# udaysankar01/xfeatSLAM

Hardware: AMD Instinct MI355X
Metric: XFeat frames/s (VGA, 4096 kpts) + 4096x4096 desc-match pairs/s (higher is better)
Workload: dtype f32

## Files before the change

xfeatslam_amd/csrc/capi.cpp:

```cpp
#include "host_stage.h"

#include <dlfcn.h>
#include <math.h>
#include <stdio.h>
#include <stdlib.h>
#include <string.h>
#include <vector>

int conv_layer_npart(int li, int Hout, int Wout);

namespace {
struct Roctx {
    int (*push)(const char*) = nullptr;
    int (*pop)() = nullptr;
};
Roctx* roctx() {
    static Roctx* R = []() -> Roctx* {
        const char* e = getenv("XFH_ROCTX");
        if (!e || !*e || *e == '0') return nullptr;
        static Roctx r;
        for (const char* n : {"librocprofiler-sdk-roctx.so.1", "librocprofiler-sdk-roctx.so", "libroctx64.so.4", "libroctx64.so"}) {
            void* h = dlopen(n, RTLD_NOW | RTLD_GLOBAL);
            if (!h) continue;
            *(void**)(&r.push) = dlsym(h, "roctxRangePushA");
// ... 136 lines not shown
            }
        }
#endif
        if (masked) {
            if (hipExtStreamCreateWithCUMask(&c->own_stream, 8, mask) != hipSuccess) return fail(XFH_ERR_HIP);
            if (hipExtStreamCreateWithCUMask(&c->aux_stream, 8, mask) != hipSuccess) return fail(XFH_ERR_HIP);
        } else {
            if (hipStreamCreateWithFlags(&c->own_stream, hipStreamNonBlocking) != hipSuccess) return fail(XFH_ERR_HIP);
            if (hipStreamCreateWithFlags(&c->aux_stream, hipStreamNonBlocking) != hipSuccess) return fail(XFH_ERR_HIP);
        }
    }
    c->stream = c->own_stream;
    if (hipEventCreateWithFlags(&c->ev_fork, hipEventDisableTiming) != hipSuccess) return fail(XFH_ERR_HIP);
    if (hipEventCreateWithFlags(&c->ev_join, hipEventDisableTiming) != hipSuccess) return fail(XFH_ERR_HIP);
    if (hipEventCreateWithFlags(&c->ev_out, hipEventDisableTiming) != hipSuccess) return fail(XFH_ERR_HIP);
    const size_t xs = (size_t)c->Hmax * c->Wmax;
    A(c->d_gray, (size_t)B * cfg->max_height * cfg->max_width);
    A(c->X, sizeof(float) * B * xs);
    c->pre_npart = (int)((xs + 1023) / 1024);
    A(c->pre_part, sizeof(double) * B * c->pre_npart * 2);
    A(c->xstat, sizeof(float) * B * 2);
    int lh[XFH_NUM_LAYERS], lw[XFH_NUM_LAYERS];
    layer_dims(c->Hmax, c->Wmax, lh, lw);
    for (int i = 0; i < XFH_NUM_LAYERS; ++i) {
        const int C = XFH_LAYERS[i].cout;
        c->raw_stride[i] = (size_t)lh[i] * lw[i] * C;
        if (i != 0) A(c->raw[i], sizeof(float) * B * c->raw_stride[i]);
        c->part_stride[i] = (size_t)conv_layer_npart(i, lh[i], lw[i]) * C * 2;
        A(c->part[i], sizeof(double) * B * c->part_stride[i]);
        A(c->stat[i], sizeof(float) * B * 2 * C);
    }
    A(c->skip_pool, sizeof(float) * B * (xs / 16));
    A(c->feats, sizeof(float) * B * c->raw_stride[17]);
    if (B > 32) { A(c->act4, sizeof(float) * B * c->raw_stride[11]); A(c->act5, sizeof(float) * B * c->raw_stride[15]); }
    A(c->feat_nrm, sizeof(float) * B * (xs / 64));
    A(c->H1, sizeof(float) * B * (xs / 64));
    A(c->K1h, sizeof(float) * B * xs);
    c->cand_cap = 1024;
    while (c->cand_cap < xs) c->cand_cap <<= 1;
    A(c->cand, sizeof(u64) * B * c->cand_cap);
    A(c->cand_count, sizeof(int) * B * CAND_CNT_STRIDE);
    A(c->slot_src, sizeof(int) * B * cfg->nfeatures);
    A(c->sel_key, sizeof(u64) * B * cfg->nfeatures);
    A(c->sel_n, sizeof(int) * B);
    const size_t rec = xfh_record_bytes(cfg->nfeatures);
    A(c->d_records, rec * B);
    if (hipHostMalloc((void**)&c->h_records, rec, hipHostMallocDefault) != hipSuccess) return fail(XFH_ERR_OUT_OF_MEMORY);
    if (hipHostMalloc((void**)&c->h_gray, (size_t)cfg->max_height * cfg->max_width, hipHostMallocDefault) != hipSuccess) return fail(XFH_ERR_OUT_OF_MEMORY);
    c->s_hgray[0] = c->h_gray; c->s_dgray[0] = c->d_gray; c->s_hrec[0] = c->h_records;
    for (int k = 1; k < xfh_ctx::SLOTS; ++k) {
        A(c->s_dgray[k], (size_t)cfg->max_height * cfg->max_width);
        if (hipHostMalloc((void**)&c->s_hgray[k], (size_t)cfg->max_height * cfg->max_width, hipHostMallocDefault) != hipSuccess) return fail(XFH_ERR_OUT_OF_MEMORY);
        if (hipHostMalloc((void**)&c->s_hrec[k], rec, hipHostMallocDefault) != hipSuccess) return fail(XFH_ERR_OUT_OF_MEMORY);
    }
    for (int k = 0; k < xfh_ctx::SLOTS; ++k)
        if (hipEventCreateWithFlags(&c->s_done[k], hipEventDisableTiming) != hipSuccess) return fail(XFH_ERR_HIP);
#undef A
    if (match_ws_reserve(c, cfg->nfeatures, cfg->nfeatures) != hipSuccess) return fail(XFH_ERR_OUT_OF_MEMORY);
    if (HostStage::reserve(c, match_mnn_stage_bytes(cfg->nfeatures, cfg->nfeatures)) != XFH_OK) return fail(XFH_ERR_OUT_OF_MEMORY);
    c->mws.cap_hout = (size_t)cfg->nfeatures * 12 + 256;
    if (hipHostMalloc((void**)&c->mws.h_out, c->mws.cap_hout, hipHostMallocDefault) != hipSuccess) return fail(XFH_ERR_OUT_OF_MEMORY);
    if (hipStreamSynchronize(c->stream) != hipSuccess) return fail(XFH_ERR_HIP);
    if (xfh_verbose()) fprintf(stderr, "[xfh] ctx %p: device %d, %dx%d (x32: %dx%d), nfeatures %d, max_batch %d, bn_mode %d, flags %d\n", (void*)c, cfg->device,
                               cfg->max_height, cfg->max_width, c->Hmax, c->Wmax, cfg->nfeatures, cfg->max_batch, cfg->bn_mode, cfg->flags);
    *out = c;
    return XFH_OK;
}

int xfh_destroy(xfh_ctx* c) {
    if (!c) return XFH_OK;
    hipSetDevice(c->cfg.device);
    if (c->twin) { xfh_destroy(c->twin); c->twin = nullptr; }
    pipe_destroy(c);
    xfh_comm_destroy(c);
    if (c->stream && c->stream != c->own_stream) hipStreamSynchronize(c->stream);
    if (c->own_stream) hipStreamSynchronize(c->own_stream);
    if (c->aux_stream) hipStreamSynchronize(c->aux_stream);
    auto F = [](void* p) { if (p) hipFree(p); };
    F(c->d_gray); F(c->X); F(c->pre_part); F(c->xstat);
    for (int i = 0; i < XFH_NUM_LAYERS; ++i) { F(c->raw[i]); F(c->part[i]); F(c->stat[i]); }
    if (!c->is_twin && !c->is_lane) {
        for (int i = 0; i < XFH_NUM_LAYERS; ++i) { F(c->w.mfma[i]); F(c->w.alt[i]); F(c->w.alt2[i]); F(c->w.m16[i]); F(c->w.bn_bias[i]); }
        for (int i = 0; i < 3; ++i) F(c->w.direct[i]);
        F(c->w.fus2); F(c->w.fus2_bias); F(c->w.skip_w); F(c->w.skip_b); F(c->w.heat2_w); F(c->w.heat2_b); F(c->w.kp3_w); F(c->w.kp3_b);
    }
    F(c->skip_pool); F(c->feats); F(c->act4); F(c->act5); F(c->feat_nrm); F(c->H1); F(c->K1h);
    F(c->cand); F(c->cand_count); F(c->slot_src); F(c->sel_key); F(c->sel_n); F(c->d_records);
    if (c->h_records) hipHostFree(c->h_records);
    if (c->h_gray) hipHostFree(c->h_gray);
    for (int k = 1; k < xfh_ctx::SLOTS; ++k) { F(c->s_dgray[k]); if (c->s_hgray[k]) hipHostFree(c->s_hgray[k]); if (c->s_hrec[k]) hipHostFree(c->s_hrec[k]); }
    for (int k = 0; k < xfh_ctx::SLOTS; ++k) if (c->s_done[k]) hipEventDestroy(c->s_done[k]);
    MatchWs& w = c->mws;
    F(w.img1); F(w.keys); F(w.stage); F(w.bkeys);
    if (w.h_out) hipHostFree(w.h_out);
    if (c->timer.ev) { for (int i = 0; i < 2 * KTimer::MAXEV; ++i) if (c->timer.ev[i]) hipEventDestroy(c->timer.ev[i]); free(c->timer.ev); }
    if (c->ev_fork) hipEventDestroy(c->ev_fork);
    if (c->ev_join) hipEventDestroy(c->ev_join);
    if (c->ev_out) hipEventDestroy(c->ev_out);
    if (c->aux_stream) hipStreamDestroy(c->aux_stream);
    if (c->own_stream) hipStreamDestroy(c->own_stream);
    delete c;
    return XFH_OK;
}

struct BlobEntry { const float* p; uint32_t dims[4]; uint32_t ndim; };
static bool blob_find(const void* blob, size_t nbytes, const char* name, BlobEntry* e) {
    const unsigned char* p = (const unsigned char*)blob;
    if (nbytes < 16 || memcmp(p, "XFHWGT01", 8) != 0) return false;
    uint32_t n; memcpy(&n, p + 8, 4);
    const size_t esz = 48 + 4 + 16 + 8;
    if (16 + (size_t)n * esz > nbytes) return false;
    const unsigned char* data = p + 16 + (size_t)n * esz;
    for (uint32_t i = 0; i < n; ++i) {
        const unsigned char* q = p + 16 + (size_t)i * esz;
        if (strncmp((const char*)q, name, 48) == 0) {
            memcpy(&e->ndim, q + 48, 4); memcpy(e->dims, q + 52, 16);
            uint64_t off; memcpy(&off, q + 68, 8);
            if (e->ndim > 4) return false;
            const uint64_t total = (nbytes - (size_t)(data - p)) / 4;
// ... 290 lines not shown
```

xfeatslam_amd/csrc/ctx.h:

```cpp
#pragma once
#include "common.h"
#include <hip/hip_ext.h>
#include <atomic>
#include <string>

struct DevWeights {
    float* direct[3] = {nullptr, nullptr, nullptr};
    float* mfma[XFH_NUM_LAYERS] = {};
    float* alt2[XFH_NUM_LAYERS] = {};
    float* m16[XFH_NUM_LAYERS] = {};
    float* alt[XFH_NUM_LAYERS] = {};
    float* bn_bias[XFH_NUM_LAYERS] = {};
    float* fus2 = nullptr;
    float* fus2_bias = nullptr;
    float* skip_w = nullptr; float* skip_b = nullptr;
    float* heat2_w = nullptr; float* heat2_b = nullptr;
    float* kp3_w = nullptr; float* kp3_b = nullptr;
    bool loaded = false;
};

struct XfhComm;
struct xfh_ctx;

#define XFH_PIPE_MAX_LANES 8
// ... 13 lines not shown
    bool inline_busy = false;
    int b_head = 0, b_count = 0;
};

struct xfh_ctx {
    xfh_config cfg;
    XfhComm* comm = nullptr;
    int Hmax = 0, Wmax = 0;
    int num_cu = 256;
    hipStream_t own_stream = nullptr;
    hipStream_t stream = nullptr;
    hipStream_t aux_stream = nullptr;
    hipEvent_t ev_fork = nullptr, ev_join = nullptr;
    hipEvent_t ev_out = nullptr;
    std::string hip_err;

    DevWeights w;

    int B = 0, H0 = 0, W0 = 0, H = 0, W = 0;
    int lh[XFH_NUM_LAYERS] = {}, lw[XFH_NUM_LAYERS] = {};
    int npart[XFH_NUM_LAYERS] = {};
    unsigned long long written[2] = {0ull, 0ull};

    uint8_t* d_gray = nullptr;
    float* X = nullptr;
    double* pre_part = nullptr; int pre_npart = 0;
    float* xstat = nullptr;
    float* raw[XFH_NUM_LAYERS] = {};
    double* part[XFH_NUM_LAYERS] = {};
    float* stat[XFH_NUM_LAYERS] = {};
    size_t raw_stride[XFH_NUM_LAYERS] = {};
    size_t part_stride[XFH_NUM_LAYERS] = {};
    float* skip_pool = nullptr; float* feats = nullptr;
    float* act4 = nullptr; float* act5 = nullptr;
    float* H1 = nullptr; float* K1h = nullptr;
    bool no_nms_heat = false;
    bool no_ride = false;
    bool select_legacy = false;
    float* feat_nrm = nullptr;
    u64* cand = nullptr; size_t cand_cap = 0;
    int* cand_count = nullptr;
    int* slot_src = nullptr;
    u64* sel_key = nullptr;
    int* sel_n = nullptr;
    uint8_t* d_records = nullptr;
    uint8_t* h_records = nullptr;
    uint8_t* h_gray = nullptr;

    static const int SLOTS = 2;
    uint8_t* s_hgray[SLOTS] = {}; uint8_t* s_dgray[SLOTS] = {}; uint8_t* s_hrec[SLOTS] = {};
    hipEvent_t s_done[SLOTS] = {};
    xfh_ctx* twin = nullptr;
    bool is_twin = false;
    int s_head = 0, s_count = 0;

    Pipe pipe;
    bool is_lane = false;

    MatchWs mws;
    KTimer timer;
};

void xfh_trace_push(const char* name);
void xfh_trace_pop();
bool xfh_verbose();
struct XfhRange { explicit XfhRange(const char* n) { xfh_trace_push(n); } ~XfhRange() { xfh_trace_pop(); } };

// ... 32 lines not shown
```

xfeatslam_amd/csrc/kernels_conv.hip:

```cpp
#include "ctx.h"
#include "heads_kp4.hip.h"
#include <stdlib.h>

struct ConvArgs {
    const float* in;
    StatSrc st;
    size_t in_stride;
    int Hin, Win;
    const float* w;
    const float* bias;
    float* out;
    size_t out_stride;
    int Hout, Wout;
    double* part;
    size_t part_stride;
    int tiles_x;
    const float* pool; size_t pool_stride; const float* skip_w; const float* skip_b;
    const float* r4; size_t s4; int H4, W4; StatSrc st4;
    const float* r5; size_t s5; int H5, W5; StatSrc st5;
    const float* xstat; const float* w0; const float* bias0;
    int dbg;
};

enum { PRO_PLAIN = 0, PRO_BN = 1, PRO_IN = 2, PRO_B2IN = 3, PRO_FUSE = 4, PRO_L0 = 5, PRO_UNFOLD = 6, PRO_FUSEA = 7  };
enum { EPI_STATS = 0, EPI_BIAS = 1, EPI_BIAS_RELU = 2 };

#ifdef XFH_STAMPS
__device__ unsigned long long g_stamps[32 * 8];
#define XFH_STAMP(a, ph) do { if (blockIdx.x == gridDim.x / 2 && blockIdx.y == 0 && blockIdx.z == 0 && threadIdx.x == 0) g_stamps[((a).dbg & 31) * 8 + (ph)] = wall_clock64(); } while (0)
extern "C" int xfh_debug_stamps(unsigned long long* out) { return (int)hipMemcpyFromSymbol(out, HIP_SYMBOL(g_stamps), sizeof g_stamps); }
#define XFH_STAMP_ROW(row, ph) do { if (blockIdx.x == gridDim.x / 2 && blockIdx.y == 0 && blockIdx.z == 0 && threadIdx.x == 0) g_stamps[(row) * 8 + (ph)] = wall_clock64(); } while (0)
#else
#define XFH_STAMP(a, ph) do { } while (0)
#define XFH_STAMP_ROW(row, ph) do { } while (0)
#endif

__device__ __forceinline__ void lin_coeff_c(int in, int out, int d, int& i0, int& i1, float& l0, float& l1) {
    const float scale = (float)in / (float)out;
    float src = fmaf(scale, (float)d + 0.5f, -0.5f);
    if (src < 0.f) src = 0.f;
    int a = (int)src;
    if (a > in - 1) a = in - 1;
    float lam = src - (float)a;
    lam = fminf(fmaxf(lam, 0.f), 1.f);
    i0 = a; i1 = a + ((a < in - 1) ? 1 : 0);
    l1 = lam; l0 = 1.f - lam;
}
template <bool ACT = false>
__device__ __forceinline__ void ld_act8(const float* __restrict__ raw, const float* st, size_t pix, int g, f32x4& v0, f32x4& v1) {
    const float* p = raw + pix * 64 + g * 8;
    v0 = *(const f32x4*)p; v1 = *(const f32x4*)(p + 4);
    if constexpr (ACT) return;
#pragma unroll
    for (int q = 0; q < 4; ++q) {
        v0[q] = fmaxf(fmaf(v0[q], st[64 + g * 8 + q], st[g * 8 + q]), 0.f);
        v1[q] = fmaxf(fmaf(v1[q], st[64 + g * 8 + 4 + q], st[g * 8 + 4 + q]), 0.f);
    }
}
template <bool ACT = false>
__device__ __forceinline__ void up_bilinear8(const float* __restrict__ raw, const float* st, int Hi, int Wi, int Ho, int Wo, int y, int x, int g, f32x4& o0, f32x4& o1) {
    int y0, y1, x0, x1; float hy0, hy1, wx0, wx1;
    lin_coeff_c(Hi, Ho, y, y0, y1, hy0, hy1);
    lin_coeff_c(Wi, Wo, x, x0, x1, wx0, wx1);
    f32x4 a0, a1, b0, b1, c0, c1, d0, d1;
    ld_act8<ACT>(raw, st, (size_t)y0 * Wi + x0, g, a0, a1); ld_act8<ACT>(raw, st, (size_t)y0 * Wi + x1, g, b0, b1);
    ld_act8<ACT>(raw, st, (size_t)y1 * Wi + x0, g, c0, c1); ld_act8<ACT>(raw, st, (size_t)y1 * Wi + x1, g, d0, d1);
#pragma unroll
    for (int j = 0; j < 4; ++j) {
        const float t0 = fmaf(wx0, a0[j], wx1 * b0[j]), u0 = fmaf(wx0, c0[j], wx1 * d0[j]);
        o0[j] = fmaf(hy0, t0, hy1 * u0);
        const float t1 = fmaf(wx0, a1[j], wx1 * b1[j]), u1 = fmaf(wx0, c1[j], wx1 * d1[j]);
        o1[j] = fmaf(hy0, t1, hy1 * u1);
    }
}

__global__ __launch_bounds__(256)
void k_act_pyramid(const float* __restrict__ raw4, size_t s4, const float* __restrict__ st4, int n4 ,
                   const float* __restrict__ raw5, size_t s5, const float* __restrict__ st5, int n5, float* __restrict__ act4, float* __restrict__ act5) {
    const int b = blockIdx.z;
    for (int q = blockIdx.x * 256 + threadIdx.x; q < (n4 + n5) / 4; q += gridDim.x * 256) {
        const bool five = q >= n4 / 4;
        const int e = (five ? q - n4 / 4 : q) * 4, ch = e & 63;
        const float* st = (five ? st5 : st4) + (size_t)b * 128;
        const size_t off = (size_t)b * (five ? s5 : s4) + e;
        f32x4 v = *(const f32x4*)((five ? raw5 : raw4) + off);
        const f32x4 be = *(const f32x4*)(st + ch), al = *(const f32x4*)(st + 64 + ch);
#pragma unroll
        for (int j = 0; j < 4; ++j) v[j] = fmaxf(fmaf(v[j], al[j], be[j]), 0.f);
        *(f32x4*)((five ? act5 : act4) + off) = v;
    }
}

__global__ __launch_bounds__(256)
void k_bn_finalize(const double* __restrict__ part, size_t part_stride, int npart, int C, double count,
                   float* __restrict__ stat ) {
    __shared__ double red[256 * 2];
    const int b = blockIdx.x;
    bn_fold<16>(part + (size_t)b * part_stride, npart, C, count, stat + (size_t)b * 2 * C, red, threadIdx.x, 256);
}

__device__ __forceinline__ double wave_sum_f64(double v) {
    v += __shfl_xor(v, 32); v += __shfl_xor(v, 16); v += __shfl_xor(v, 8);
    v += __shfl_xor(v, 4); v += __shfl_xor(v, 2); v += __shfl_xor(v, 1);
    return v;
}
typedef float f32x2 __attribute__((ext_vector_type(2)));
__device__ __forceinline__ void l0_conv(const float (&win)[9], const XFH_CONST float* __restrict__ w, float (&acc)[4]) {
    f32x2 a0 = {0.f, 0.f}, a1 = {0.f, 0.f};
#pragma unroll
    for (int k = 0; k < 9; ++k) {
        const f32x2 v = {win[k], win[k]};
        a0 = __builtin_elementwise_fma(v, f32x2{w[k * 4], w[k * 4 + 1]}, a0);
        a1 = __builtin_elementwise_fma(v, f32x2{w[k * 4 + 2], w[k * 4 + 3]}, a1);
    }
    acc[0] = a0.x; acc[1] = a0.y; acc[2] = a1.x; acc[3] = a1.y;
}

constexpr int L0S_TW = 128, L0S_TH = 32, L0S_R = 4;
__global__ __launch_bounds__(256)
void k_block1_stats(const float* __restrict__ X, size_t x_stride, StatSrc xs, int H, int W, int tiles_x,
                    const float* __restrict__ w0, double* __restrict__ part, size_t part_stride, float* __restrict__ pool, size_t pool_stride) {
    __shared__ double s_red[512];
    __shared__ float s_xst[2];
// ... 304 lines not shown
            if (cok && prow < rows_left && pcol + 4 * h < cols_left) value(n, r, dst, bv);
        }
    }
}

#ifndef XFH_PD
#define XFH_PD 3
#endif

template <int CIN, int COUT, int KS, int ST, int WM, int WN, int NT, int WW, int PRO, int EPI, int CBMAX = 64, int TPC = 1, int PD = XFH_PD>
__device__ __forceinline__ void conv_mfma_body(const ConvArgs a, const int tile, const int b, float* smem) {
    constexpr int NTHR = 64 * WM * WN;
    constexpr int WH = 32 / WW, TH = WM * WH, TW = WW;
    constexpr int COUTP = WN * NT * 32;
    constexpr int PAD = KS / 2;
    constexpr int TIH = (TH - 1) * ST + KS, TIW = (TW - 1) * ST + KS;
    constexpr int CP = CIN + 4;
    constexpr int CB = CIN > CBMAX ? CBMAX : CIN;
    constexpr int NCB = CIN / CB;
    static_assert(TPC == 1 || NCB == 1, "several taps per chunk only with all channels in the chunk");
    static_assert((KS * KS) % TPC == 0, "taps per chunk");
    constexpr int NCHUNK = KS * KS * NCB / TPC;
    constexpr int NWBUF = NCHUNK > 1 ? 2 : 1;
    constexpr int KC = TPC * CB;
    constexpr int WS = KC + 4;
    constexpr int WCH = COUTP * KC;
    constexpr int NWLD = (WCH / 4 + NTHR - 1) / NTHR;
    constexpr int G = CIN / 8;
    constexpr int IN_FLOATS = TIH * TIW * CP;
    constexpr int W_FLOATS = COUTP * WS;

    float* s_in = smem;
    float* s_w = smem + IN_FLOATS;
    float* s_stat = s_w + NWBUF * W_FLOATS;

    const int t = threadIdx.x;
    const int tx0 = (tile % a.tiles_x) * TW, ty0 = (tile / a.tiles_x) * TH;
    const float* in = a.in + (size_t)b * a.in_stride;

    XFH_STAMP(a, 0);
    f32x4 wreg[PD][NWLD];
    const __amdgpu_buffer_rsrc_t wrs = wbuf_make(a.w);
#pragma unroll
    for (int c = 0; c < PD; ++c)
#pragma unroll
        for (int q = 0; q < NWLD; ++q) {
            const int f = t + q * NTHR;
            if (c < NCHUNK && f < WCH / 4) wreg[c][q] = wbuf_ld(wrs, f, c * WCH);
        }
    constexpr int NITEM = TIH * TIW * G;
    constexpr int NIT = (NITEM + NTHR - 1) / NTHR;
    constexpr bool FUSE = PRO == PRO_FUSE || PRO == PRO_FUSEA;
    constexpr bool BATCHED = !FUSE;
    f32x4 r0[BATCHED ? NIT : 1], r1[BATCHED ? NIT : 1];
    float rp[PRO == PRO_B2IN ? NIT : 1];
    if constexpr (BATCHED) {
#pragma unroll
        for (int k = 0; k < NIT; ++k) {
            const int item = t + k * NTHR, pix = item / G, g = item % G;
            const int gy = min(max(ty0 * ST - PAD + pix / TIW, 0), a.Hin - 1), gx = min(max(tx0 * ST - PAD + pix % TIW, 0), a.Win - 1);
            const float* p = PRO == PRO_UNFOLD ? in + ((size_t)(gy * 8 + g) * (a.Win * 8) + gx * 8) : in + ((size_t)gy * a.Win + gx) * CIN + g * 8;
            r0[k] = *(const f32x4*)p;
            r1[k] = *(const f32x4*)(p + 4);
            if constexpr (PRO == PRO_B2IN) rp[k] = a.pool[(size_t)b * a.pool_stride + (size_t)gy * a.Win + gx];
        }
    }
    XFH_STAMP(a, 1);
    if constexpr (PRO == PRO_BN || PRO == PRO_B2IN || FUSE) stage_stat(a.st, b, CIN, tile == 0, s_stat, (double*)s_in, t, NTHR);
    if constexpr (PRO == PRO_B2IN) {
        for (int q = t; q < CIN; q += NTHR) { s_stat[2 * CIN + q] = a.skip_w[q]; s_stat[3 * CIN + q] = a.skip_b[q]; }
        __syncthreads();
    }
    if constexpr (PRO == PRO_FUSE) {
        stage_stat(a.st4, b, 64, tile == 0, s_stat + 128, (double*)s_in, t, NTHR);
        stage_stat(a.st5, b, 64, tile == 0, s_stat + 256, (double*)s_in, t, NTHR);
    }
    XFH_STAMP(a, 2);
    if constexpr (BATCHED) {
#pragma unroll
        for (int k = 0; k < NIT; ++k) {
            const int item = t + k * NTHR, pix = item / G, g = item % G;
            const int gy = ty0 * ST - PAD + pix / TIW, gx = tx0 * ST - PAD + pix % TIW;
            const bool ok = gy >= 0 && gy < a.Hin && gx >= 0 && gx < a.Win;
            if (NITEM % NTHR != 0 && item >= NITEM) continue;
            f32x4 v0 = r0[k], v1 = r1[k];
            if constexpr (PRO == PRO_UNFOLD) {
                const float xm = a.xstat[b * 2], xr = a.xstat[b * 2 + 1];
#pragma unroll
                for (int q = 0; q < 4; ++q) { v0[q] = fmaf(v0[q], xr, xm); v1[q] = fmaf(v1[q], xr, xm); }
            }
            if constexpr (PRO == PRO_BN || PRO == PRO_B2IN) {
                const f32x4 m0 = *(const f32x4*)(s_stat + g * 8), m1 = *(const f32x4*)(s_stat + g * 8 + 4);
                const f32x4 q0 = *(const f32x4*)(s_stat + CIN + g * 8), q1 = *(const f32x4*)(s_stat + CIN + g * 8 + 4);
#pragma unroll
                for (int q = 0; q < 4; ++q) {
                    v0[q] = fmaxf(fmaf(v0[q], q0[q], m0[q]), 0.f);
                    v1[q] = fmaxf(fmaf(v1[q], q1[q], m1[q]), 0.f);
                }
            }
            if constexpr (PRO == PRO_B2IN) {
                const float pl = rp[k];
#pragma unroll
                for (int q = 0; q < 4; ++q) {
                    v0[q] = v0[q] + (pl * s_stat[2 * CIN + g * 8 + q] + s_stat[3 * CIN + g * 8 + q]);
                    v1[q] = v1[q] + (pl * s_stat[2 * CIN + g * 8 + 4 + q] + s_stat[3 * CIN + g * 8 + 4 + q]);
                }
            }
            if constexpr (KS > 1) { if (!ok) { v0 = f32x4{0.f, 0.f, 0.f, 0.f}; v1 = v0; } }
            float* d = s_in + pix * CP + g * 8;
            *(f32x4*)d = f32x4{v0.x, v0.z, v1.x, v1.z};
            *(f32x4*)(d + 4) = f32x4{v0.y, v0.w, v1.y, v1.w};
        }
    } else
    for (int item = t; item < TIH * TIW * G; item += NTHR) {
        const int pix = item / G, g = item % G;
        const int iy = pix / TIW, ix = pix % TIW;
        const int gy = ty0 * ST - PAD + iy, gx = tx0 * ST - PAD + ix;
        f32x4 v0 = {0.f, 0.f, 0.f, 0.f}, v1 = {0.f, 0.f, 0.f, 0.f};
        if (gy >= 0 && gy < a.Hin && gx >= 0 && gx < a.Win) {
            const float* p = in + ((size_t)gy * a.Win + gx) * CIN + g * 8;
            v0 = *(const f32x4*)p;
            v1 = *(const f32x4*)(p + 4);
#pragma unroll
            for (int q = 0; q < 4; ++q) {
                v0[q] = fmaxf(fmaf(v0[q], s_stat[CIN + g * 8 + q], s_stat[g * 8 + q]), 0.f);
                v1[q] = fmaxf(fmaf(v1[q], s_stat[CIN + g * 8 + 4 + q], s_stat[g * 8 + 4 + q]), 0.f);
            }
            f32x4 u0, u1, w0, w1;
            up_bilinear8<PRO == PRO_FUSEA>(a.r4 + (size_t)b * a.s4, s_stat + 128, a.H4, a.W4, a.Hin, a.Win, gy, gx, g, u0, u1);
            up_bilinear8<PRO == PRO_FUSEA>(a.r5 + (size_t)b * a.s5, s_stat + 256, a.H5, a.W5, a.Hin, a.Win, gy, gx, g, w0, w1);
#pragma unroll
            for (int q = 0; q < 4; ++q) { v0[q] = (v0[q] + u0[q]) + w0[q]; v1[q] = (v1[q] + u1[q]) + w1[q]; }
        }
        float* d = s_in + pix * CP + g * 8;
        *(f32x4*)d = f32x4{v0.x, v0.z, v1.x, v1.z};
        *(f32x4*)(d + 4) = f32x4{v0.y, v0.w, v1.y, v1.w};
    }
#pragma unroll
    for (int q = 0; q < NWLD; ++q) {
        const int f = t + q * NTHR;
        if (f < WCH / 4) {
            const int n = f / (KC / 4), c4 = f % (KC / 4);
            *(f32x4*)(s_w + n * WS + c4 * 4) = wreg[0][q];
            if (PD < NCHUNK) wreg[0][q] = wbuf_ld(wrs, f, PD * WCH);
        }
    }
    __syncthreads();
    XFH_STAMP(a, 3);

    const int wave = __builtin_amdgcn_readfirstlane(t >> 6), lane = t & 63, i = lane & 31, h = lane >> 5;
    const int wm = wave / WN, wn = wave % WN;
    const int pr = i / WW, pc = i % WW;
    const int ly = (wm * WH + pr) * ST, lx = pc * ST;

    float biasv[NT];
    conv_bias<COUT, NT, EPI>(a.bias, wn * NT * 32 + i, biasv);
    f32x16 acc[NT];
#pragma unroll
    for (int n = 0; n < NT; ++n)
#pragma unroll
        for (int r = 0; r < 16; ++r) acc[n][r] = 0.f;

#pragma unroll
    for (int ch = 0; ch < NCHUNK; ++ch) {
#pragma unroll
        for (int tt = 0; tt < TPC; ++tt) {
            const int tap = TPC == 1 ? ch / NCB : ch * TPC + tt, cb = TPC == 1 ? ch % NCB : 0;
            const int ky = tap / KS, kx = tap % KS;
            const float* pa = s_in + ((ly + ky) * TIW + lx + kx) * CP + cb * CB + 4 * h;
// ... 802 lines not shown
                sum[n] += __shfl_xor(sum[n], 32);
                sq[n] += __shfl_xor(sq[n], 32);
                if (h == 0) {
                    const int co = n * 32 + i;
                    s_red[(wm * COUTP + co) * 2 + 0] = sum[n];
                    s_red[(wm * COUTP + co) * 2 + 1] = sq[n];
                }
            }
        }
        __syncthreads();
        if constexpr (EPI == EPI_STATS) {
            for (int co = t; co < COUT; co += NTHR) {
                double S = 0.0, SS = 0.0;
#pragma unroll
                for (int m = 0; m < WM; ++m) { S += s_red[(m * COUTP + co) * 2 + 0]; SS += s_red[(m * COUTP + co) * 2 + 1]; }
                double* p = a.part + (size_t)b * a.part_stride + ((size_t)tl * COUT + co) * 2;
                p[0] = S; p[1] = SS;
            }
        }
        if (!has_next) break;
        store_tile(next);
        __syncthreads();
        tile = next;
    }
}

template <int CIN, int COUT, int KS, int ST, int WM, int WN, int NT, int WW, int PRO, int EPI, int CBMAX = 64, int TPC = 1>
static hipError_t conv_mfma_launch(xfh_ctx* c, const ConvArgs& a, int B, int* npart_out, int layer) {
    constexpr int WH = 32 / WW, TH = WM * WH, TW = WW;
    constexpr int COUTP = WN * NT * 32;
    constexpr int TIH = (TH - 1) * ST + KS, TIW = (TW - 1) * ST + KS;
    constexpr int CB = CIN > CBMAX ? CBMAX : CIN;
    constexpr int NWBUF = (KS * KS * (CIN / CB) / TPC) > 1 ? 2 : 1;
    constexpr int STATF = (PRO == PRO_FUSE || PRO == PRO_FUSEA) ? 384 : (PRO == PRO_B2IN ? 4 * CIN : 2 * CIN);
    constexpr size_t LDS = sizeof(float) * ((size_t)TIH * TIW * (CIN + 4) + NWBUF * (size_t)COUTP * (TPC * CB + 4) + STATF);
    static_assert(LDS <= 160 * 1024, "LDS budget");
    static_assert(sizeof(double) * WM * COUTP * 2 <= LDS, "stat scratch");
    static_assert(sizeof(double) * 512 <= sizeof(float) * (size_t)TIH * TIW * (CIN + 4), "bn_fold scratch in the input tile");
    ConvArgs aa = a;
    aa.dbg = layer;
    aa.tiles_x = (a.Wout + TW - 1) / TW;
    const int tiles_y = (a.Hout + TH - 1) / TH;
    const int ntile = aa.tiles_x * tiles_y;
    if (npart_out) *npart_out = ntile;
    auto kern = k_conv_mfma<CIN, COUT, KS, ST, WM, WN, NT, WW, PRO, EPI, CBMAX, TPC>;
    XFH_SET_LDS_ATTR_ONCE(c, kern, LDS);
    launch_k(c, XFH_K_CONV_MFMA, layer, kern, dim3(ntile, 1, B), dim3(64 * WM * WN), LDS, aa);
    return hipGetLastError();
}

#ifndef XFH_CONV_T
#define XFH_CONV_T 1
#endif
template <int CIN, int COUT, int KS, int ST, int WM, int WN, int NT, int WW, int PRO, int EPI, int CBMAX = 64>
static hipError_t conv_mfma_t_launch(xfh_ctx* c, const ConvArgs& a, int B, int* npart_out, int layer) {
    constexpr int WH = 32 / WW, TH = WM * WH, TW = WW;
    constexpr int COUTP = WN * NT * 32;
    constexpr int TIH = (TH - 1) * ST + KS, TIW = (TW - 1) * ST + KS;
    constexpr int CB = CIN > CBMAX ? CBMAX : CIN;
    constexpr size_t LDS = sizeof(float) * ((size_t)TIH * TIW * (CIN + 4) + 3 * (size_t)COUTP * (CB + 4)) + sizeof(double) * WM * COUTP * 2;
    static_assert(LDS <= 160 * 1024, "LDS budget");
    ConvArgs aa = a;
    aa.dbg = layer;
    aa.tiles_x = (a.Wout + TW - 1) / TW;
    const int ntile = aa.tiles_x * ((a.Hout + TH - 1) / TH);
    if (npart_out) *npart_out = ntile;
    auto kern = k_conv_mfma_t<CIN, COUT, KS, ST, WM, WN, NT, WW, PRO, EPI, CBMAX>;
    XFH_SET_LDS_ATTR_ONCE(c, kern, LDS);
    const int total = ntile * B;
// ... 115 lines not shown
            a.xstat = c->xstat; a.w0 = c->w.direct[0]; a.bias0 = (EPI == EPI_BIAS_RELU) ? c->w.bn_bias[0] : nullptr;
            e = conv_direct_launch<4, 8, 2, PRO_L0>(c, a, B, &np, li);
            break;
        case 2: e = conv_direct_launch<8, 8, 1, PRO_BN>(c, a, B, &np, li); break;
        case 3:
            a.w = c->w.alt[li];
            if (persistent(B)) e = conv_mfma_p_launch<8, 24, 3, 2, 4, 1, 1, 16, PRO_BN, EPI>(c, a, B, &np, li);
            else e = conv_mfma_launch<8, 24, 3, 2, 4, 1, 1, 16, PRO_BN, EPI, 64, 9>(c, a, B, &np, li);
            break;
        case 4:
            if (persistent(B)) { a.w = c->w.alt[li]; e = conv_mfma_p_launch<24, 24, 3, 1, 4, 1, 1, 16, PRO_B2IN, EPI>(c, a, B, &np, li); }
            else { a.w = c->w.alt[li]; e = conv_mfma_launch<24, 24, 3, 1, 4, 1, 1, 16, PRO_B2IN, EPI, 64, 9>(c, a, B, &np, li); }
            break;
        case 5:
            if (persistent(B)) { a.w = c->w.alt[li]; e = conv_mfma_p_launch<24, 24, 3, 1, 4, 1, 1, 16, PRO_BN, EPI>(c, a, B, &np, li); }
            else { a.w = c->w.alt[li]; e = conv_mfma_launch<24, 24, 3, 1, 4, 1, 1, 16, PRO_BN, EPI, 64, 9>(c, a, B, &np, li); }
            break;
        case 6:
            if (consumer_fold(B)) { a.w = c->w.alt[li]; e = conv_mfma_launch<24, 64, 3, 2, 4, 1, 2, 16, PRO_BN, EPI, 64, 3>(c, a, B, &np, li); }
            else if constexpr ((XFH_CONV_T & 2) != 0) { if (!small_batch(B)) e = conv_mfma_t_launch<24, 64, 3, 2, 4, 1, 2, 16, PRO_BN, EPI>(c, a, B, &np, li); else e = conv_mfma_launch<24, 64, 3, 2, 4, 1, 2, 16, PRO_BN, EPI>(c, a, B, &np, li); }
            else e = conv_mfma_launch<24, 64, 3, 2, 4, 1, 2, 16, PRO_BN, EPI>(c, a, B, &np, li);
            break;
        case 7: case 17: case 16:
            if (small_batch(B)) {
                a.w = c->w.m16[li];
                const long t2 = (long)((Hout + 1) / 2) * ((Wout + 15) / 16) * B;
                if (li == 16) e = split_channels(Hout, Wout, 2, 16, B) ? conv_mfma16_launch<64, 64, 1, 16, 2, PRO_FUSE, EPI, 2>(c, a, B, &np, li)
                                : t2 > XFH_M16_TALL ? conv_mfma16_launch<64, 64, 1, 16, 4, PRO_FUSE, EPI>(c, a, B, &np, li) : conv_mfma16_launch<64, 64, 1, 16, 2, PRO_FUSE, EPI>(c, a, B, &np, li);
                else e = split_channels(Hout, Wout, 2, 16, B) ? conv_mfma16_launch<64, 64, 1, 16, 2, PRO_BN, EPI, 2>(c, a, B, &np, li)
                       : t2 > XFH_M16_TALL ? conv_mfma16_launch<64, 64, 1, 16, 4, PRO_BN, EPI>(c, a, B, &np, li) : conv_mfma16_launch<64, 64, 1, 16, 2, PRO_BN, EPI>(c, a, B, &np, li);
            } else {
                a.w = c->w.alt[li];
                if (li == 16) {
                    const int n4 = c->lh[11] * c->lw[11] * 64, n5 = c->lh[15] * c->lw[15] * 64;
                    hipLaunchKernelGGL(k_act_pyramid, dim3(((n4 + n5) / 4 + 255) / 256, 1, B), dim3(256), 0, c->stream, (const float*)c->raw[11], c->raw_stride[11],
                                       (const float*)c->stat[11], n4, (const float*)c->raw[15], c->raw_stride[15], (const float*)c->stat[15], n5, c->act4, c->act5);
                    a.r4 = c->act4; a.r5 = c->act5;
                    e = conv_mfma_launch<64, 64, 3, 1, 4, 2, 1, 16, PRO_FUSEA, EPI, 32>(c, a, B, &np, li);
                }
                else if constexpr ((XFH_CONV_T & 16) != 0) e = conv_mfma_t_launch<64, 64, 3, 1, 4, 2, 1, 16, PRO_BN, EPI, 32>(c, a, B, &np, li);
                else e = conv_mfma_launch<64, 64, 3, 1, 4, 2, 1, 16, PRO_BN, EPI, 32>(c, a, B, &np, li);
            }
            break;
        case 8:
            if (persistent(B)) e = conv_mfma_p_launch<64, 64, 1, 1, 4, 1, 2, 16, PRO_BN, EPI>(c, a, B, &np, li);
            else e = conv_mfma_launch<64, 64, 1, 1, 4, 1, 2, 16, PRO_BN, EPI>(c, a, B, &np, li);
            break;
        case 9:
            if (small_batch(B)) { a.w = c->w.m16[li]; e = split_channels(Hout, Wout, 4, 8, B) ? conv_mfma16_launch<64, 64, 2, 8, 2, PRO_BN, EPI, 2>(c, a, B, &np, li) : conv_mfma16_launch<64, 64, 2, 8, 2, PRO_BN, EPI>(c, a, B, &np, li); }
            else if constexpr ((XFH_CONV_T & 1) != 0) e = conv_mfma_t_launch<64, 64, 3, 2, 2, 2, 1, 8, PRO_BN, EPI>(c, a, B, &np, li);
            else e = conv_mfma_launch<64, 64, 3, 2, 2, 2, 1, 8, PRO_BN, EPI>(c, a, B, &np, li);
            break;
        case 10: case 11:
            if (small_batch(B)) { a.w = c->w.m16[li]; e = split_channels(Hout, Wout, 4, 8, B) ? conv_mfma16_launch<64, 64, 1, 8, 2, PRO_BN, EPI, 2>(c, a, B, &np, li) : conv_mfma16_launch<64, 64, 1, 8, 2, PRO_BN, EPI>(c, a, B, &np, li); }
            else if constexpr ((XFH_CONV_T & 4) != 0) { a.w = c->w.alt[li]; e = conv_mfma_t_launch<64, 64, 3, 1, 4, 2, 1, 8, PRO_BN, EPI, 32>(c, a, B, &np, li); }
            else { a.w = c->w.alt[li]; e = conv_mfma_launch<64, 64, 3, 1, 4, 2, 1, 8, PRO_BN, EPI, 32>(c, a, B, &np, li); }
            break;
        case 12:
            if (small_batch(B)) { a.w = c->w.m16[li]; e = split_channels(Hout, Wout, 4, 4, B) ? conv_mfma16_launch<64, 128, 2, 4, 1, PRO_BN, EPI, 2>(c, a, B, &np, li) : conv_mfma16_launch<64, 128, 2, 4, 1, PRO_BN, EPI>(c, a, B, &np, li); break; }
            a.w = c->w.alt[li];
            if constexpr ((XFH_CONV_T & 2) != 0) e = conv_mfma_t_launch<64, 128, 3, 2, 1, 4, 1, 8, PRO_BN, EPI, 32>(c, a, B, &np, li);
            else e = conv_mfma_launch<64, 128, 3, 2, 1, 4, 1, 8, PRO_BN, EPI, 32>(c, a, B, &np, li);
            break;
        case 13: case 14:
            if constexpr ((XFH_CONV_T & 8) != 0) { if (!small_batch(B)) { a.w = c->w.alt[li]; e = conv_mfma_t_launch<128, 128, 3, 1, 4, 4, 1, 8, PRO_BN, EPI, 32>(c, a, B, &np, li); break; } }
            if (!small_batch(B)) { a.w = c->w.alt[li]; e = conv_mfma_launch<128, 128, 3, 1, 4, 4, 1, 8, PRO_BN, EPI, 32>(c, a, B, &np, li); }
            else { a.w = c->w.m16[li]; e = split_channels(Hout, Wout, 4, 4, B) ? conv_mfma16_launch<128, 128, 1, 4, 1, PRO_BN, EPI, 2>(c, a, B, &np, li) : conv_mfma16_launch<128, 128, 1, 4, 1, PRO_BN, EPI>(c, a, B, &np, li); }
            break;
        case 15: e = conv_mfma_launch<128, 64, 1, 1, 1, 2, 1, 8, PRO_BN, EPI>(c, a, B, &np, li); break;
        case 18:
            if (persistent(B)) e = conv_mfma_p_launch<64, 64, 1, 1, 4, 1, 2, 16, PRO_PLAIN, EPI>(c, a, B, &np, li);
// ... 200 lines not shown
```

Measured before the change: 32590.

## Fuse pyramid BN-ReLU into fusion conv via LDS patches, drop act_pyramid pass

Removes the separate k_act_pyramid kernel and its act4/act5 buffers for large batches. The fusion conv (layer 16) now loads a small per-tile patch of the coarser pyramid levels, applies BN+ReLU once into LDS, and does the bilinear upsampling from LDS. It also software-pipelines the global input loads one step ahead. This saves a full-tensor read/write round trip and a kernel launch, at the cost of extra LDS use and a hard requirement that the levels be exact 2x/4x downsamples.

```diff
diff --git a/xfeatslam_amd/csrc/capi.cpp b/xfeatslam_amd/csrc/capi.cpp
--- a/xfeatslam_amd/csrc/capi.cpp
+++ b/xfeatslam_amd/csrc/capi.cpp
@@ -192,7 +192,6 @@
     }
     A(c->skip_pool, sizeof(float) * B * (xs / 16));
     A(c->feats, sizeof(float) * B * c->raw_stride[17]);
-    if (B > 32) { A(c->act4, sizeof(float) * B * c->raw_stride[11]); A(c->act5, sizeof(float) * B * c->raw_stride[15]); }
     A(c->feat_nrm, sizeof(float) * B * (xs / 64));
     A(c->H1, sizeof(float) * B * (xs / 64));
     A(c->K1h, sizeof(float) * B * xs);
@@ -244,7 +243,7 @@
         for (int i = 0; i < 3; ++i) F(c->w.direct[i]);
         F(c->w.fus2); F(c->w.fus2_bias); F(c->w.skip_w); F(c->w.skip_b); F(c->w.heat2_w); F(c->w.heat2_b); F(c->w.kp3_w); F(c->w.kp3_b);
     }
-    F(c->skip_pool); F(c->feats); F(c->act4); F(c->act5); F(c->feat_nrm); F(c->H1); F(c->K1h);
+    F(c->skip_pool); F(c->feats); F(c->feat_nrm); F(c->H1); F(c->K1h);
     F(c->cand); F(c->cand_count); F(c->slot_src); F(c->sel_key); F(c->sel_n); F(c->d_records);
     if (c->h_records) hipHostFree(c->h_records);
     if (c->h_gray) hipHostFree(c->h_gray);
diff --git a/xfeatslam_amd/csrc/ctx.h b/xfeatslam_amd/csrc/ctx.h
--- a/xfeatslam_amd/csrc/ctx.h
+++ b/xfeatslam_amd/csrc/ctx.h
@@ -69,7 +69,6 @@
     size_t raw_stride[XFH_NUM_LAYERS] = {};
     size_t part_stride[XFH_NUM_LAYERS] = {};
     float* skip_pool = nullptr; float* feats = nullptr;
-    float* act4 = nullptr; float* act5 = nullptr;
     float* H1 = nullptr; float* K1h = nullptr;
     bool no_nms_heat = false;
     bool no_ride = false;
diff --git a/xfeatslam_amd/csrc/kernels_conv.hip b/xfeatslam_amd/csrc/kernels_conv.hip
--- a/xfeatslam_amd/csrc/kernels_conv.hip
+++ b/xfeatslam_amd/csrc/kernels_conv.hip
@@ -22,7 +22,7 @@
     int dbg;
 };
 
-enum { PRO_PLAIN = 0, PRO_BN = 1, PRO_IN = 2, PRO_B2IN = 3, PRO_FUSE = 4, PRO_L0 = 5, PRO_UNFOLD = 6, PRO_FUSEA = 7  };
+enum { PRO_PLAIN = 0, PRO_BN = 1, PRO_IN = 2, PRO_B2IN = 3, PRO_FUSE = 4, PRO_L0 = 5, PRO_UNFOLD = 6, PRO_FUSEP = 7  };
 enum { EPI_STATS = 0, EPI_BIAS = 1, EPI_BIAS_RELU = 2 };
 
 #ifdef XFH_STAMPS
@@ -46,25 +46,22 @@
     i0 = a; i1 = a + ((a < in - 1) ? 1 : 0);
     l1 = lam; l0 = 1.f - lam;
 }
-template <bool ACT = false>
 __device__ __forceinline__ void ld_act8(const float* __restrict__ raw, const float* st, size_t pix, int g, f32x4& v0, f32x4& v1) {
     const float* p = raw + pix * 64 + g * 8;
     v0 = *(const f32x4*)p; v1 = *(const f32x4*)(p + 4);
-    if constexpr (ACT) return;
 #pragma unroll
     for (int q = 0; q < 4; ++q) {
         v0[q] = fmaxf(fmaf(v0[q], st[64 + g * 8 + q], st[g * 8 + q]), 0.f);
         v1[q] = fmaxf(fmaf(v1[q], st[64 + g * 8 + 4 + q], st[g * 8 + 4 + q]), 0.f);
     }
 }
-template <bool ACT = false>
 __device__ __forceinline__ void up_bilinear8(const float* __restrict__ raw, const float* st, int Hi, int Wi, int Ho, int Wo, int y, int x, int g, f32x4& o0, f32x4& o1) {
     int y0, y1, x0, x1; float hy0, hy1, wx0, wx1;
     lin_coeff_c(Hi, Ho, y, y0, y1, hy0, hy1);
     lin_coeff_c(Wi, Wo, x, x0, x1, wx0, wx1);
     f32x4 a0, a1, b0, b1, c0, c1, d0, d1;
-    ld_act8<ACT>(raw, st, (size_t)y0 * Wi + x0, g, a0, a1); ld_act8<ACT>(raw, st, (size_t)y0 * Wi + x1, g, b0, b1);
-    ld_act8<ACT>(raw, st, (size_t)y1 * Wi + x0, g, c0, c1); ld_act8<ACT>(raw, st, (size_t)y1 * Wi + x1, g, d0, d1);
+    ld_act8(raw, st, (size_t)y0 * Wi + x0, g, a0, a1); ld_act8(raw, st, (size_t)y0 * Wi + x1, g, b0, b1);
+    ld_act8(raw, st, (size_t)y1 * Wi + x0, g, c0, c1); ld_act8(raw, st, (size_t)y1 * Wi + x1, g, d0, d1);
 #pragma unroll
     for (int j = 0; j < 4; ++j) {
         const float t0 = fmaf(wx0, a0[j], wx1 * b0[j]), u0 = fmaf(wx0, c0[j], wx1 * d0[j]);
@@ -74,21 +71,34 @@
     }
 }
 
-__global__ __launch_bounds__(256)
-void k_act_pyramid(const float* __restrict__ raw4, size_t s4, const float* __restrict__ st4, int n4 ,
-                   const float* __restrict__ raw5, size_t s5, const float* __restrict__ st5, int n5, float* __restrict__ act4, float* __restrict__ act5) {
-    const int b = blockIdx.z;
-    for (int q = blockIdx.x * 256 + threadIdx.x; q < (n4 + n5) / 4; q += gridDim.x * 256) {
-        const bool five = q >= n4 / 4;
-        const int e = (five ? q - n4 / 4 : q) * 4, ch = e & 63;
-        const float* st = (five ? st5 : st4) + (size_t)b * 128;
-        const size_t off = (size_t)b * (five ? s5 : s4) + e;
-        f32x4 v = *(const f32x4*)((five ? raw5 : raw4) + off);
-        const f32x4 be = *(const f32x4*)(st + ch), al = *(const f32x4*)(st + 64 + ch);
-#pragma unroll
-        for (int j = 0; j < 4; ++j) v[j] = fmaxf(fmaf(v[j], al[j], be[j]), 0.f);
-        *(f32x4*)((five ? act5 : act4) + off) = v;
-    }
+constexpr int FP_H4 = 6, FP_W4 = 10, FP_H5 = 4, FP_W5 = 6;
+constexpr int FP_CELLS4 = FP_H4 * FP_W4, FP_CELLS = FP_CELLS4 + FP_H5 * FP_W5;
+constexpr int FP_CS = 68;
+constexpr int FP_FLOATS = FP_CELLS * FP_CS;
+__device__ __forceinline__ int fuse_patch_origin(int in, int out, int d0) {
+    int i0, i1; float l0, l1;
+    lin_coeff_c(in, out, max(d0, 0), i0, i1, l0, l1);
+    return i0;
+}
+struct PatchTaps { int o00, o01, o10, o11; float wx0, wx1, hy0, hy1; };
+template <int PW>
+__device__ __forceinline__ PatchTaps patch_taps(int py, int px, int Hi, int Wi, int Ho, int Wo, int y, int x) {
+    int y0, y1, x0, x1; PatchTaps k;
+    lin_coeff_c(Hi, Ho, y, y0, y1, k.hy0, k.hy1);
+    lin_coeff_c(Wi, Wo, x, x0, x1, k.wx0, k.wx1);
+    k.o00 = ((y0 - py) * PW + x0 - px) * FP_CS; k.o01 = ((y0 - py) * PW + x1 - px) * FP_CS;
+    k.o10 = ((y1 - py) * PW + x0 - px) * FP_CS; k.o11 = ((y1 - py) * PW + x1 - px) * FP_CS;
+    return k;
+}
+__device__ __forceinline__ f32x4 patch_blend4(const float* patch , const PatchTaps& k) {
+    const f32x4 a = *(const f32x4*)(patch + k.o00), b = *(const f32x4*)(patch + k.o01), c = *(const f32x4*)(patch + k.o10), d = *(const f32x4*)(patch + k.o11);
+    f32x4 o;
+#pragma unroll
+    for (int j = 0; j < 4; ++j) {
+        const float t = fmaf(k.wx0, a[j], k.wx1 * b[j]), u = fmaf(k.wx0, c[j], k.wx1 * d[j]);
+        o[j] = fmaf(k.hy0, t, k.hy1 * u);
+    }
+    return o;
 }
 
 __global__ __launch_bounds__(256)
@@ -459,7 +469,11 @@
 
     float* s_in = smem;
     float* s_w = smem + IN_FLOATS;
-    float* s_stat = s_w + NWBUF * W_FLOATS;
+    constexpr bool FUSE = PRO == PRO_FUSEP;
+    static_assert(!FUSE || (CIN == 64 && KS == 3 && ST == 1 && NCHUNK > 1 && TH % 4 == 0 && TW % 4 == 0 && TIH / 2 + 1 == FP_H4 && TIW / 2 + 1 == FP_W4 && TIH / 4 + 2 == FP_H5 && TIW / 4 + 2 == FP_W5),
+                  "the patch extents are derived for this tile");
+    float* s_patch = s_w;
+    float* s_stat = s_w + (FUSE && FP_FLOATS > NWBUF * W_FLOATS ? FP_FLOATS : NWBUF * W_FLOATS);
 
     const int t = threadIdx.x;
     const int tx0 = (tile % a.tiles_x) * TW, ty0 = (tile / a.tiles_x) * TH;
@@ -477,10 +491,30 @@
         }
     constexpr int NITEM = TIH * TIW * G;
     constexpr int NIT = (NITEM + NTHR - 1) / NTHR;
-    constexpr bool FUSE = PRO == PRO_FUSE || PRO == PRO_FUSEA;
     constexpr bool BATCHED = !FUSE;
     f32x4 r0[BATCHED ? NIT : 1], r1[BATCHED ? NIT : 1];
     float rp[PRO == PRO_B2IN ? NIT : 1];
+    constexpr int NPL = FUSE ? (FP_CELLS * 16 + NTHR - 1) / NTHR : 1;
+    f32x4 pv[NPL];
+    int py4 = 0, px4 = 0, py5 = 0, px5 = 0;
+    if constexpr (FUSE) {
+        py4 = fuse_patch_origin(a.H4, a.Hin, ty0 - PAD); px4 = fuse_patch_origin(a.W4, a.Win, tx0 - PAD);
+        py5 = fuse_patch_origin(a.H5, a.Hin, ty0 - PAD); px5 = fuse_patch_origin(a.W5, a.Win, tx0 - PAD);
+#pragma unroll
+        for (int q = 0; q < NPL; ++q) {
+            const int f = t + q * NTHR, cell = min(f >> 4, FP_CELLS - 1);
+            const bool five = cell >= FP_CELLS4;
+            const int cy = five ? (cell - FP_CELLS4) / FP_W5 : cell / FP_W4, cx = five ? (cell - FP_CELLS4) % FP_W5 : cell % FP_W4;
+            const int sy = min((five ? py5 : py4) + cy, (five ? a.H5 : a.H4) - 1), sx = min((five ? px5 : px4) + cx, (five ? a.W5 : a.W4) - 1);
+            const float* p = (five ? a.r5 + (size_t)b * a.s5 : a.r4 + (size_t)b * a.s4) + ((size_t)sy * (five ? a.W5 : a.W4) + sx) * 64 + (f & 15) * 4;
+            pv[q] = *(const f32x4*)p;
+        }
+        const int pix = t / G;
+        const int gy = min(max(ty0 - PAD + pix / TIW, 0), a.Hin - 1), gx = min(max(tx0 - PAD + pix % TIW, 0), a.Win - 1);
+        const float* p = in + ((size_t)gy * a.Win + gx) * CIN + (t % G) * 8;
+        r0[0] = *(const f32x4*)p;
+        r1[0] = *(const f32x4*)(p + 4);
+    }
     if constexpr (BATCHED) {
 #pragma unroll
         for (int k = 0; k < NIT; ++k) {
@@ -493,14 +527,26 @@
         }
     }
     XFH_STAMP(a, 1);
+    if constexpr (FUSE)
+        for (int q = t; q < 256; q += NTHR) s_stat[128 + q] = q < 128 ? a.st4.stat[(size_t)b * 128 + q] : a.st5.stat[(size_t)b * 128 + q - 128];
     if constexpr (PRO == PRO_BN || PRO == PRO_B2IN || FUSE) stage_stat(a.st, b, CIN, tile == 0, s_stat, (double*)s_in, t, NTHR);
     if constexpr (PRO == PRO_B2IN) {
         for (int q = t; q < CIN; q += NTHR) { s_stat[2 * CIN + q] = a.skip_w[q]; s_stat[3 * CIN + q] = a.skip_b[q]; }
         __syncthreads();
     }
-    if constexpr (PRO == PRO_FUSE) {
-        stage_stat(a.st4, b, 64, tile == 0, s_stat + 128, (double*)s_in, t, NTHR);
-        stage_stat(a.st5, b, 64, tile == 0, s_stat + 256, (double*)s_in, t, NTHR);
+    if constexpr (FUSE) {
+#pragma unroll
+        for (int q = 0; q < NPL; ++q) {
+            const int f = t + q * NTHR, cell = f >> 4, c4 = (f & 15) * 4;
+            if (FP_CELLS * 16 % NTHR != 0 && cell >= FP_CELLS) continue;
+            const float* st = s_stat + (cell >= FP_CELLS4 ? 256 : 128);
+            const f32x4 be = *(const f32x4*)(st + c4), al = *(const f32x4*)(st + 64 + c4);
+            f32x4 v = pv[q];
+#pragma unroll
+            for (int j = 0; j < 4; ++j) v[j] = fmaxf(fmaf(v[j], al[j], be[j]), 0.f);
+            *(f32x4*)(s_patch + cell * FP_CS + c4) = v;
+        }
+        __syncthreads();
     }
     XFH_STAMP(a, 2);
     if constexpr (BATCHED) {
@@ -538,30 +584,37 @@
             *(f32x4*)d = f32x4{v0.x, v0.z, v1.x, v1.z};
             *(f32x4*)(d + 4) = f32x4{v0.y, v0.w, v1.y, v1.w};
         }
-    } else
-    for (int item = t; item < TIH * TIW * G; item += NTHR) {
-        const int pix = item / G, g = item % G;
-        const int iy = pix / TIW, ix = pix % TIW;
-        const int gy = ty0 * ST - PAD + iy, gx = tx0 * ST - PAD + ix;
-        f32x4 v0 = {0.f, 0.f, 0.f, 0.f}, v1 = {0.f, 0.f, 0.f, 0.f};
-        if (gy >= 0 && gy < a.Hin && gx >= 0 && gx < a.Win) {
-            const float* p = in + ((size_t)gy * a.Win + gx) * CIN + g * 8;
-            v0 = *(const f32x4*)p;
-            v1 = *(const f32x4*)(p + 4);
+    } else {
+#pragma unroll 1
+        for (int item = t; item < NITEM; item += NTHR) {
+            const int pix = item / G, g = item % G;
+            const int gy = ty0 - PAD + pix / TIW, gx = tx0 - PAD + pix % TIW;
+            const bool ok = gy >= 0 && gy < a.Hin && gx >= 0 && gx < a.Win;
+            const int cy = min(max(gy, 0), a.Hin - 1), cx = min(max(gx, 0), a.Win - 1);
+            f32x4 v0 = r0[0], v1 = r1[0];
+            {
+                const int npix = (item + NTHR) / G;
+                const int ny = min(max(ty0 - PAD + npix / TIW, 0), a.Hin - 1), nx = min(max(tx0 - PAD + npix % TIW, 0), a.Win - 1);
+                const float* p = in + ((size_t)ny * a.Win + nx) * CIN + g * 8;
+                r0[0] = *(const f32x4*)p;
+                r1[0] = *(const f32x4*)(p + 4);
+            }
+            const f32x4 m0 = *(const f32x4*)(s_stat + g * 8), m1 = *(const f32x4*)(s_stat + g * 8 + 4);
+            const f32x4 q0 = *(const f32x4*)(s_stat + CIN + g * 8), q1 = *(const f32x4*)(s_stat + CIN + g * 8 + 4);
+            const PatchTaps k4 = patch_taps<FP_W4>(py4, px4, a.H4, a.W4, a.Hin, a.Win, cy, cx), k5 = patch_taps<FP_W5>(py5, px5, a.H5, a.W5, a.Hin, a.Win, cy, cx);
+            const float* p4 = s_patch + g * 8, * p5 = s_patch + FP_CELLS4 * FP_CS + g * 8;
+            const f32x4 u0 = patch_blend4(p4, k4), w0 = patch_blend4(p5, k5), u1 = patch_blend4(p4 + 4, k4), w1 = patch_blend4(p5 + 4, k5);
 #pragma unroll
             for (int q = 0; q < 4; ++q) {
-                v0[q] = fmaxf(fmaf(v0[q], s_stat[CIN + g * 8 + q], s_stat[g * 8 + q]), 0.f);
-                v1[q] = fmaxf(fmaf(v1[q], s_stat[CIN + g * 8 + 4 + q], s_stat[g * 8 + 4 + q]), 0.f);
-            }
-            f32x4 u0, u1, w0, w1;
-            up_bilinear8<PRO == PRO_FUSEA>(a.r4 + (size_t)b * a.s4, s_stat + 128, a.H4, a.W4, a.Hin, a.Win, gy, gx, g, u0, u1);
-            up_bilinear8<PRO == PRO_FUSEA>(a.r5 + (size_t)b * a.s5, s_stat + 256, a.H5, a.W5, a.Hin, a.Win, gy, gx, g, w0, w1);
-#pragma unroll
-            for (int q = 0; q < 4; ++q) { v0[q] = (v0[q] + u0[q]) + w0[q]; v1[q] = (v1[q] + u1[q]) + w1[q]; }
-        }
-        float* d = s_in + pix * CP + g * 8;
-        *(f32x4*)d = f32x4{v0.x, v0.z, v1.x, v1.z};
-        *(f32x4*)(d + 4) = f32x4{v0.y, v0.w, v1.y, v1.w};
+                v0[q] = (fmaxf(fmaf(v0[q], q0[q], m0[q]), 0.f) + u0[q]) + w0[q];
+                v1[q] = (fmaxf(fmaf(v1[q], q1[q], m1[q]), 0.f) + u1[q]) + w1[q];
+            }
+            if (!ok) { v0 = f32x4{0.f, 0.f, 0.f, 0.f}; v1 = v0; }
+            float* d = s_in + pix * CP + g * 8;
+            *(f32x4*)d = f32x4{v0.x, v0.z, v1.x, v1.z};
+            *(f32x4*)(d + 4) = f32x4{v0.y, v0.w, v1.y, v1.w};
+        }
+        __syncthreads();
     }
 #pragma unroll
     for (int q = 0; q < NWLD; ++q) {
@@ -1430,9 +1483,11 @@
     constexpr int TIH = (TH - 1) * ST + KS, TIW = (TW - 1) * ST + KS;
     constexpr int CB = CIN > CBMAX ? CBMAX : CIN;
     constexpr int NWBUF = (KS * KS * (CIN / CB) / TPC) > 1 ? 2 : 1;
-    constexpr int STATF = (PRO == PRO_FUSE || PRO == PRO_FUSEA) ? 384 : (PRO == PRO_B2IN ? 4 * CIN : 2 * CIN);
-    constexpr size_t LDS = sizeof(float) * ((size_t)TIH * TIW * (CIN + 4) + NWBUF * (size_t)COUTP * (TPC * CB + 4) + STATF);
+    constexpr int STATF = PRO == PRO_FUSEP ? 384 : (PRO == PRO_B2IN ? 4 * CIN : 2 * CIN);
+    constexpr size_t WF = NWBUF * (size_t)COUTP * (TPC * CB + 4);
+    constexpr size_t LDS = sizeof(float) * ((size_t)TIH * TIW * (CIN + 4) + (PRO == PRO_FUSEP && (size_t)FP_FLOATS > WF ? (size_t)FP_FLOATS : WF) + STATF);
     static_assert(LDS <= 160 * 1024, "LDS budget");
+    static_assert(PRO != PRO_FUSEP || LDS <= 80 * 1024, "block_fusion.0 with its patches: two workgroups per CU");
     static_assert(sizeof(double) * WM * COUTP * 2 <= LDS, "stat scratch");
     static_assert(sizeof(double) * 512 <= sizeof(float) * (size_t)TIH * TIW * (CIN + 4), "bn_fold scratch in the input tile");
     ConvArgs aa = a;
@@ -1614,11 +1669,8 @@
             } else {
                 a.w = c->w.alt[li];
                 if (li == 16) {
-                    const int n4 = c->lh[11] * c->lw[11] * 64, n5 = c->lh[15] * c->lw[15] * 64;
-                    hipLaunchKernelGGL(k_act_pyramid, dim3(((n4 + n5) / 4 + 255) / 256, 1, B), dim3(256), 0, c->stream, (const float*)c->raw[11], c->raw_stride[11],
-                                       (const float*)c->stat[11], n4, (const float*)c->raw[15], c->raw_stride[15], (const float*)c->stat[15], n5, c->act4, c->act5);
-                    a.r4 = c->act4; a.r5 = c->act5;
-                    e = conv_mfma_launch<64, 64, 3, 1, 4, 2, 1, 16, PRO_FUSEA, EPI, 32>(c, a, B, &np, li);
+                    if (a.H4 * 2 != Hin || a.W4 * 2 != Win || a.H5 * 4 != Hin || a.W5 * 4 != Win) return hipErrorInvalidValue;
+                    e = conv_mfma_launch<64, 64, 3, 1, 4, 2, 1, 16, PRO_FUSEP, EPI, 32>(c, a, B, &np, li);
                 }
                 else if constexpr ((XFH_CONV_T & 16) != 0) e = conv_mfma_t_launch<64, 64, 3, 1, 4, 2, 1, 16, PRO_BN, EPI, 32>(c, a, B, &np, li);
                 else e = conv_mfma_launch<64, 64, 3, 1, 4, 2, 1, 16, PRO_BN, EPI, 32>(c, a, B, &np, li);
```

Result: no change. 32910 (median of 6 runs) (+1.0%).
